# glmanhtu/vit-ed

Measured on AMD Instinct MI355X. Metric: patch-pairs/sec fwd+bwd, div2k_erosion7_4bin_patch8_64 ViT-ED, higher is better.
Workload: dtype bf16

## Files before the change

include/vited.h:

```cpp
#ifndef VITED_H
#define VITED_H

#include <stdint.h>

#ifdef __cplusplus
extern "C" {
#endif

#define VITED_ABI_VERSION 1

#define VITED_OK 0
#define VITED_ERR_BAD_ARG 1
#define VITED_ERR_UNSUPPORTED 2
#define VITED_ERR_LAUNCH 3
#define VITED_ERR_WORKSPACE 4

#define VITED_F32 0
#define VITED_BF16 1
#define VITED_F16 2
#define VITED_I32 3
#define VITED_I64 4

#define VITED_EPI_STORE 0
#define VITED_EPI_GELU 1
// ... 67 lines not shown
int64_t vited_layernorm_bwd_workspace_bytes(int64_t rows, int64_t dim);
int vited_layernorm_bwd(const void* dy, int dy_dtype, int64_t dy_ld, const float* x, int64_t x_ld,
                        const float* gamma, const float* mean, const float* rstd, const float* dx_in,
                        int64_t dx_in_ld, float* dx_out, int64_t dx_out_ld, void* dx_lp, int dx_lp_dtype,
                        int64_t dx_lp_ld, float* dgamma, float* dbeta, int accumulate, int64_t rows, int64_t dim,
                        float* workspace, int64_t workspace_bytes, void* stream);

int vited_layernorm_bwd_scaled(const void* dy, int dy_dtype, int64_t dy_ld, const float* x, int64_t x_ld,
                               const float* gamma, const float* mean, const float* rstd, const float* dx_in,
                               int64_t dx_in_ld, float* dx_out, int64_t dx_out_ld, void* dx_lp, int dx_lp_dtype,
                               int64_t dx_lp_ld, const float* lp_scale, float* dgamma, float* dbeta, int accumulate,
                               int64_t rows, int64_t dim, float* workspace, int64_t workspace_bytes, void* stream);

int vited_scale_rows_cast(const float* src, int64_t src_ld, const float* row_scale, void* dst, int dst_dtype, int64_t dst_ld,
                          int64_t rows, int64_t dim, void* stream);


int vited_gemm(const void* A, int64_t lda, const void* B, int64_t ldb, int b_layout, int dtype, int64_t M,
               int64_t N, int64_t K, int epilogue, const float* bias, const void* aux,
               const float* residual, void* out, void* out2, int64_t ldo, int64_t rows_per_batch,
               int64_t out_rows_per_batch, int64_t row_offset, int residual_bcast, void* stream);

int vited_gemm_scaled(const void* A, int64_t lda, const void* B, int64_t ldb, int b_layout, int dtype, int64_t M, int64_t N,
                      int64_t K, const float* bias, const float* residual, const float* row_scale, float* out, int64_t ldo,
                      void* stream);

int64_t vited_linear_bwd_weight_workspace_bytes(int64_t M, int64_t N, int64_t K);
int vited_linear_bwd_weight(const void* dY, int64_t lddy, const void* X, int64_t ldx, int dtype, int64_t M,
                            int64_t N, int64_t K, float* dW, float* dbias, int accumulate, float* workspace,
                            int64_t workspace_bytes, void* stream);

int vited_linear_bwd_weight_batched_supported(int count, const int64_t* M, const int64_t* N, const int64_t* K, int dtype);
int64_t vited_linear_bwd_weight_batched_workspace_bytes(int count, const int64_t* M, const int64_t* N, const int64_t* K);
int vited_linear_bwd_weight_batched(int count, const void* const* dY, const int64_t* lddy, const void* const* X,
                                    const int64_t* ldx, const int64_t* M, const int64_t* N, const int64_t* K, float* const* dW,
                                    float* const* dbias, int dtype, int accumulate, float* workspace, int64_t workspace_bytes,
                                    void* stream);

int vited_linear_layernorm_supported(int64_t M, int64_t N, int64_t K);

int vited_linear_residual_layernorm_fwd(const void* a, int64_t lda, const void* w, int64_t ldw, const float* bias,
                                        const float* residual, int64_t ldr, float* y, int64_t ldy, const float* gamma,
                                        const float* beta, float eps, void* h, int64_t ldh, float* mean, float* rstd,
                                        int64_t M, int64_t N, int64_t K, void* stream);

int vited_linear_residual_layernorm_fwd_scaled(const void* a, int64_t lda, const void* w, int64_t ldw, const float* bias,
                                               const float* residual, int64_t ldr, const float* row_scale, float* y, int64_t ldy,
                                               const float* gamma, const float* beta, float eps, void* h, int64_t ldh, float* mean,
                                               float* rstd, int64_t M, int64_t N, int64_t K, void* stream);

int vited_linear_layernorm_bwd_segmented(const void* dy, int64_t lddy, int64_t seg_k, int64_t seg_stride, int64_t segments,
                                         const void* wt, int64_t ldwt, const float* x, int64_t ldx, const float* gamma,
                                         const float* mean, const float* rstd, const float* dx_in, int64_t dx_in_ld,
                                         float* dx_out, int64_t dx_out_ld, void* dx_lp, int64_t dx_lp_ld, float* dgamma,
                                         float* dbeta, int accumulate, int64_t M, int64_t N, float* workspace,
                                         int64_t workspace_bytes, void* stream);
int64_t vited_linear_layernorm_bwd_partial_rows(int64_t M);
int vited_layernorm_bwd_finish_batched(int count, const float* const* partial, const int* nparts, float* const* dgamma,
                                       float* const* dbeta, const int* accumulate, int64_t dim, void* stream);
int64_t vited_linear_layernorm_bwd_workspace_bytes(int64_t M, int64_t N);
int vited_linear_layernorm_bwd(const void* dy, int64_t lddy, const void* wt, int64_t ldwt, const float* x, int64_t ldx,
                               const float* gamma, const float* mean, const float* rstd, const float* dx_in,
                               int64_t dx_in_ld, float* dx_out, int64_t dx_out_ld, void* dx_lp, int64_t dx_lp_ld,
                               float* dgamma, float* dbeta, int accumulate, int64_t M, int64_t N, int64_t K,
                               float* workspace, int64_t workspace_bytes, void* stream);

// ... 114 lines not shown
```

vit-ed_amd/csrc/gemm.hip:

```cpp
#include <stdlib.h>
#include <string.h>

#include "gemm_kernels.h"

static thread_local int g_last_gemm_path = 0;
extern "C" int vited_last_gemm_path(void) { return g_last_gemm_path; }

static int gemm_impl(const void* A, int64_t lda, const void* B, int64_t ldb, int b_layout, int dtype, int64_t M, int64_t N, int64_t K,
                     int epilogue, const float* bias, const void* aux, const float* residual, void* out, void* out2, int64_t ldo,
                     int64_t rows_per_batch, int64_t out_rows_per_batch, int64_t row_offset, int residual_bcast,
                     const float* row_scale, void* stream) {
    if (!A || !B || !out || M <= 0 || N <= 0 || K <= 0 || lda < K || ldo < N) return VITED_ERR_BAD_ARG;
    if (b_layout != VITED_B_NK && b_layout != VITED_B_KN) return VITED_ERR_BAD_ARG;
    if (ldb < (b_layout == VITED_B_NK ? K : N)) return VITED_ERR_BAD_ARG;
    if (epilogue < VITED_EPI_STORE || epilogue > VITED_EPI_GELU_GRAD) return VITED_ERR_BAD_ARG;
    if ((epilogue == VITED_EPI_GELU || epilogue == VITED_EPI_GELU_GRAD) && !out2) return VITED_ERR_BAD_ARG;
    if (epilogue == VITED_EPI_RESIDUAL && !residual) return VITED_ERR_BAD_ARG;
    if ((epilogue == VITED_EPI_MUL_GELU_GRAD || epilogue == VITED_EPI_MUL) && !aux) return VITED_ERR_BAD_ARG;
    if (rows_per_batch < 0 || (rows_per_batch > 0 && (out_rows_per_batch < rows_per_batch + row_offset || row_offset < 0)))
        return VITED_ERR_BAD_ARG;
    if (row_scale) {
        if (epilogue != VITED_EPI_RESIDUAL || rows_per_batch != 0) return VITED_ERR_BAD_ARG;
        epilogue = EPI_RESIDUAL_SCALED;
    }
// ... 75 lines not shown
        return rc;
    }
    g_last_gemm_path = 1;
    rc = gemm_tn_portable(dY, lddy, X, ldx, dtype, M, N, K, splits, slab, s);
    if (rc != VITED_OK) return rc;
    if (via_slabs) {
        rc = sum_rows_f32_single_pass(workspace, N * K, dW, splits, N * K, s, accumulate);
        if (rc != VITED_OK) return rc;
    }
    if (dbias) {
        float* ws2 = bias_tmp + N;
        const int64_t ws2_bytes = workspace_bytes - (splits * N * K + N) * (int64_t)sizeof(float);
        if (accumulate) {
            rc = vited_sum_rows(dY, dtype, lddy, bias_tmp, M, N, ws2, ws2_bytes, stream);
            if (rc == VITED_OK) rc = sum_rows_f32_single_pass(bias_tmp, N, dbias, 1, N, s, 1);
        } else {
            rc = vited_sum_rows(dY, dtype, lddy, dbias, M, N, ws2, ws2_bytes, stream);
        }
    }
    return rc;
}

extern "C" int vited_linear_bwd_weight_batched_supported(int count, const int64_t* M, const int64_t* N, const int64_t* K, int dtype) {
    return dtype == VITED_BF16 && gemm_tn_batch_supported(count, M, N, K) ? 1 : 0;
}

extern "C" int64_t vited_linear_bwd_weight_batched_workspace_bytes(int count, const int64_t* M, const int64_t* N, const int64_t* K) {
    if (!gemm_tn_batch_supported(count, M, N, K)) return 0;
    int64_t splits, ws, bs;
    gemm_tn_batch_layout(count, M, N, K, &splits, &ws, &bs);
    return splits * (ws + bs) * (int64_t)sizeof(float) + 256;
}

extern "C" int vited_linear_bwd_weight_batched(int count, const void* const* dY, const int64_t* lddy, const void* const* X,
                                               const int64_t* ldx, const int64_t* M, const int64_t* N, const int64_t* K,
                                               float* const* dW, float* const* dbias, int dtype, int accumulate, float* workspace,
                                               int64_t workspace_bytes, void* stream) {
    if (count < 1 || !dY || !lddy || !X || !ldx || !M || !N || !K || !dW || !dbias || !workspace) return VITED_ERR_BAD_ARG;
    if (dtype != VITED_BF16 || !gemm_tn_batch_supported(count, M, N, K)) return VITED_ERR_UNSUPPORTED;
    if (workspace_bytes < vited_linear_bwd_weight_batched_workspace_bytes(count, M, N, K)) return VITED_ERR_WORKSPACE;
    int64_t splits, ws, bs;
    gemm_tn_batch_layout(count, M, N, K, &splits, &ws, &bs);
    int has_bias[40];
    int64_t widths[40], nbias[40];
    for (int i = 0; i < count; ++i) {
        if (!dY[i] || !X[i] || !dW[i] || lddy[i] < N[i] || ldx[i] < K[i]) return VITED_ERR_BAD_ARG;
        has_bias[i] = dbias[i] != nullptr;
        widths[i] = N[i] * K[i];
        nbias[i] = N[i];
    }
    float* base = (float*)(((uintptr_t)workspace + 15) & ~(uintptr_t)15);
    float* slabs = base;
    float* bias_slabs = base + splits * ws;
    hipStream_t s = (hipStream_t)stream;
    g_last_gemm_path = 2;
    int rc = gemm_tn_batch(count, dY, lddy, X, ldx, M, N, K, has_bias, slabs, bias_slabs, s);
    if (rc != VITED_OK) return rc;
    return sum_slabs_batch(count, slabs, ws, bias_slabs, bs, splits, widths, dW, nbias, dbias, accumulate, s);
}
```

vit-ed_amd/csrc/gemm_kernels.h:

```cpp
#pragma once
#include "gemm_epilogue.h"

int gemm_portable(const void* A, int64_t lda, const void* B, int64_t ldb, int b_layout, int dtype, int64_t M, int64_t N,
                  int64_t K, int epilogue, const EpiParams& ep, hipStream_t s);
int gemm_tn_portable(const void* dY, int64_t lddy, const void* X, int64_t ldx, int dtype, int64_t M, int64_t N, int64_t K,
                     int64_t splits, float* out, hipStream_t s);

bool gemm_nt_mfma_supported(const void* A, int64_t lda, const void* B, int64_t ldb, int64_t M, int64_t N, int64_t K,
                            int epilogue, const EpiParams& ep);
int gemm_nt_mfma(const void* A, int64_t lda, const void* B, int64_t ldb, int64_t M, int64_t N, int64_t K, int epilogue,
                 const EpiParams& ep, hipStream_t s);
bool gemm_nt_areg_supported(int64_t ldw, int64_t M, int64_t N, int64_t K, int epilogue);
int gemm_nt_areg(const void* A, int64_t lda, const void* W, int64_t ldw, int64_t M, int64_t N, int epilogue, int waves,
                 const EpiParams& ep, hipStream_t s);
bool gemm_tn_mfma_supported(const void* dY, int64_t lddy, const void* X, int64_t ldx, int64_t M, int64_t N, int64_t K);
int64_t gemm_tn_mfma_splits(int64_t M, int64_t N, int64_t K);
int gemm_tn_mfma(const void* dY, int64_t lddy, const void* X, int64_t ldx, int64_t M, int64_t N, int64_t K, int64_t splits,
                 float* out, float* bias_out , hipStream_t s);

bool gemm_tn_batch_supported(int count, const int64_t* M, const int64_t* N, const int64_t* K);
void gemm_tn_batch_layout(int count, const int64_t* M, const int64_t* N, const int64_t* K, int64_t* splits, int64_t* slab_stride,
                          int64_t* bias_stride);
int gemm_tn_batch(int count, const void* const* dY, const int64_t* lddy, const void* const* X, const int64_t* ldx, const int64_t* M,
                  const int64_t* N, const int64_t* K, const int* has_bias, float* slabs, float* bias_slabs, hipStream_t s);
int sum_slabs_batch(int count, const float* slabs, int64_t slab_stride, const float* bias_slabs, int64_t bias_stride, int64_t splits,
                    const int64_t* widths, float* const* dW, const int64_t* nbias, float* const* dbias, int accumulate, hipStream_t s);

int sum_rows_f32_single_pass(const float* in, int64_t in_ld, float* out, int64_t batch, int64_t width, hipStream_t s,
                             int accumulate = 0);
int sum_slabs_pair(const float* in_a, int64_t ld_a, float* out_a, int64_t width_a, const float* in_b, int64_t ld_b, float* out_b,
                   int64_t width_b, int64_t batch, hipStream_t s, int accumulate);
```

vit-ed_amd/csrc/gemm_mfma.hip:

```cpp
#include <stdlib.h>

#include <mutex>

#include "gemm_kernels.h"
#include "gemm_nt_epilogue.h"
#include "gemm_lds.h"

template <int BKT, int WM, bool ASM_DMA = false>
__device__ __forceinline__ void nt_stage_load(const bf16* __restrict__ A, int64_t lda, const bf16* __restrict__ B,
                                              int64_t ldb, int64_t m0, int64_t n0, int64_t M, int64_t N, int64_t k0,
                                              char* stage, int wave, int lane) {
    using C = NtCfg<BKT, WM>;
    const int rsub = lane / C::CHUNKS, cp = lane % C::CHUNKS;
#ifndef NT_DBG_NO_A_DMA
#pragma unroll
    for (int i = 0; i < 32 / C::ROWS_PER_DMA; ++i) {
        const int r = wave * 32 + i * C::ROWS_PER_DMA + rsub;
        const int c = cp ^ C::swz(r);
        int64_t gm = m0 + r;
        gm = gm < M ? gm : M - 1;
        const bf16* asrc = A + gm * lda + k0 + c * 8;
        if constexpr (ASM_DMA) glds16_asm(asrc, stage + (wave * 32 + i * C::ROWS_PER_DMA) * C::ROW_BYTES);
        else glds16(asrc, stage + (wave * 32 + i * C::ROWS_PER_DMA) * C::ROW_BYTES);
    }
// ... 750 lines not shown
        status = hipFuncSetAttribute((const void*)gemm_tn_wide_kernel<true>, hipFuncAttributeMaxDynamicSharedMemorySize, LDS);
        if (status == hipSuccess)
            status = hipFuncSetAttribute((const void*)gemm_tn_wide_kernel<false>, hipFuncAttributeMaxDynamicSharedMemorySize, LDS);
    });
    if (status != hipSuccess) return VITED_ERR_LAUNCH;
    if (any_bias)
        hipLaunchKernelGGL((gemm_tn_wide_kernel<true>), dim3(b.total_tiles, (unsigned)splits), dim3(512), LDS, s, b, out, bias_out);
    else
        hipLaunchKernelGGL((gemm_tn_wide_kernel<false>), dim3(b.total_tiles, (unsigned)splits), dim3(512), LDS, s, b, out, bias_out);
    return VITED_OK;
}

static int launch_tn_wide(const void* dY, int64_t lddy, const void* X, int64_t ldx, int64_t M, int64_t N, int64_t K, int64_t splits,
                          float* out, float* bias_out, hipStream_t s) {
    TwBatch b = {};
    TwProblem& p = b.p[0];
    p.dY = (const bf16*)dY; p.X = (const bf16*)X; p.lddy = lddy; p.ldx = ldx; p.M = M;
    p.rows_per_split = ceil_div64(ceil_div64(M, splits), 32) * 32;
    p.N = (int)N; p.K = (int)K; p.tiles_k = (int)(K / 384); p.tile0 = 0; p.has_bias = bias_out != nullptr;
    b.count = 1;
    b.total_tiles = (int)ceil_div64(N, 128) * p.tiles_k;
    b.slab_stride = N * K;
    b.bias_stride = N;
    return launch_tn_wide_batch(b, splits, bias_out != nullptr, out, bias_out, s);
}

bool gemm_tn_batch_supported(int count, const int64_t* M, const int64_t* N, const int64_t* K) {
    if (count < 1 || count > TW_MAX_PROBLEMS) return false;
    for (int i = 0; i < count; ++i)
        if (!tn_use_wide(M[i], N[i], K[i]) || N[i] % 8 || N[i] > (1 << 20) || K[i] > (1 << 20)) return false;
    return true;
}

static inline int64_t tn_batch_splits(int count, const int64_t* M, const int64_t* N, const int64_t* K) {
    int64_t tiles = 0, mmin = M[0];
    for (int i = 0; i < count; ++i) {
        tiles += ceil_div64(N[i], 128) * (K[i] / 384);
        mmin = M[i] < mmin ? M[i] : mmin;
    }
    int64_t s = 256 / tiles;
    const int64_t max_s = ceil_div64(mmin, 256);
    if (s > max_s) s = max_s;
    return s < 1 ? 1 : s;
}

void gemm_tn_batch_layout(int count, const int64_t* M, const int64_t* N, const int64_t* K, int64_t* splits, int64_t* slab_stride,
                          int64_t* bias_stride) {
    *splits = tn_batch_splits(count, M, N, K);
    int64_t w = 0, b = 0;
    for (int i = 0; i < count; ++i) {
        w += N[i] * K[i];
        b += N[i];
    }
    *slab_stride = w;
    *bias_stride = b;
}

int gemm_tn_batch(int count, const void* const* dY, const int64_t* lddy, const void* const* X, const int64_t* ldx, const int64_t* M,
                  const int64_t* N, const int64_t* K, const int* has_bias, float* slabs, float* bias_slabs, hipStream_t s) {
    TwBatch b = {};
    int64_t splits;
    gemm_tn_batch_layout(count, M, N, K, &splits, &b.slab_stride, &b.bias_stride);
    int tile = 0;
    int64_t woff = 0, boff = 0;
    bool any_bias = false;
    for (int i = 0; i < count; ++i) {
        TwProblem& p = b.p[i];
        if (!gemm_tn_mfma_supported(dY[i], lddy[i], X[i], ldx[i], M[i], N[i], K[i])) return VITED_ERR_UNSUPPORTED;
        p.dY = (const bf16*)dY[i]; p.X = (const bf16*)X[i]; p.lddy = lddy[i]; p.ldx = ldx[i]; p.M = M[i];
        p.rows_per_split = ceil_div64(ceil_div64(M[i], splits), 32) * 32;
        p.N = (int)N[i]; p.K = (int)K[i]; p.tiles_k = (int)(K[i] / 384); p.tile0 = tile; p.has_bias = has_bias[i];
        p.slab_off = woff; p.bias_off = boff;
        tile += (int)ceil_div64(N[i], 128) * p.tiles_k;
        woff += N[i] * K[i];
        boff += N[i];
        any_bias = any_bias || has_bias[i];
    }
    b.count = count;
    b.total_tiles = tile;
    const int rc = launch_tn_wide_batch(b, splits, any_bias, slabs, bias_slabs, s);
    return rc != VITED_OK ? rc : vited_check_launch();
}

int gemm_tn_mfma(const void* dY, int64_t lddy, const void* X, int64_t ldx, int64_t M, int64_t N, int64_t K, int64_t splits,
                 float* out, float* bias_out, hipStream_t s) {
    int rc;
    if (tn_use_wide(M, N, K)) rc = launch_tn_wide(dY, lddy, X, ldx, M, N, K, splits, out, bias_out, s);
#if TN_FORCE_TM
    else rc = launch_tn<TN_FORCE_TM, TN_FORCE_STAGES>(dY, lddy, X, ldx, M, N, K, splits, out, bias_out, s);
#else
    else if (tn_use_ring(M, N, K)) rc = launch_tn<32, 3>(dY, lddy, X, ldx, M, N, K, splits, out, bias_out, s);
    else rc = launch_tn<64, 2>(dY, lddy, X, ldx, M, N, K, splits, out, bias_out, s);
#endif
    return rc != VITED_OK ? rc : vited_check_launch();
}
```

vit-ed_amd/functions.py:

```python
from __future__ import annotations

import contextlib
import os
from collections import namedtuple

import torch

from . import ops
from ._lib import (B_KN, B_NK, EPI_GELU_GRAD, EPI_MUL, EPI_RESIDUAL, EPI_STORE, EPI_STORE_F32)

LN_EPS = 1e-6


def _bundle(name, table):
    fields, keys = zip(*(pair.split('=') for pair in table.split()))
    return namedtuple(name, fields), keys


_ATTN = 'g1=norm1.weight b1=norm1.bias wqkv=attn.qkv.weight bqkv=attn.qkv.bias wproj=attn.proj.weight bproj=attn.proj.bias '
_CROSS = ('gc=norm_cross.weight bc=norm_cross.bias gx=norm_context.weight bx=norm_context.bias wq=cross_attn.q.weight '
          'bq=cross_attn.q.bias wkv=cross_attn.kv.weight bkv=cross_attn.kv.bias wcp=cross_attn.proj.weight bcp=cross_attn.proj.bias ')
_MLP = 'g2=norm2.weight b2=norm2.bias w1=mlp.fc1.weight bb1=mlp.fc1.bias w2=mlp.fc2.weight bb2=mlp.fc2.bias'
_PATCH = 'pw=patch_embed.proj.weight pb=patch_embed.proj.bias pos=pos_embed '
EncBlock, ENC_BLOCK_KEYS = _bundle('EncBlock', _ATTN + _MLP)
DecBlock, DEC_BLOCK_KEYS = _bundle('DecBlock', _ATTN + _CROSS + _MLP)
EncShared, ENC_SHARED_KEYS = _bundle('EncShared', _PATCH)
DecShared, DEC_SHARED_KEYS = _bundle('DecShared', _PATCH + 'cls=cls_token gN=norm.weight bN=norm.bias wh=head.weight bh=head.bias')


def split_params(params, shared_type, block_type):
    ns, nb = len(shared_type._fields), len(block_type._fields)
    if len(params) < ns or (len(params) - ns) % nb:
        raise ValueError(f'{len(params)} parameters are not {ns} shared + a whole number of {nb}-parameter blocks')
    return shared_type._make(params[:ns]), [block_type._make(params[i: i + nb]) for i in range(ns, len(params), nb)]


def flatten_params(shared, blocks):
# ... 150 lines not shown
        return tuple(self.get(i, j) for j in range(self.per_sample.shape[1]))


def _take_drop_rows(rt, which, nblk, nbr, batch, n, device, cls_block=None):
    dp = rt.drop_path
    if dp is None or dp[which] is None:
        return None
    scales, live = dp[which], dp[2][which]
    if not any(any(row) for row in live):
        return None
    if tuple(scales.shape) != (nblk, nbr, batch) or scales.dtype != torch.float32 or scales.device != device:
        raise ValueError(f'drop-path scales: expected fp32 {(nblk, nbr, batch)} on {device}, got {scales.dtype} {tuple(scales.shape)} on '
                         f'{scales.device}')
    return _DropRows(scales.contiguous(), live, n, cls_block)


def _gtarget(rt, p):
    if p is None or not rt.direct_grads:
        return None
    g = p.grad
    if g is None or g.dtype != torch.float32 or not g.is_contiguous() or g.shape != p.shape or g.device != p.device:
        return None
    return g


def _ln_bwd(rt, dy, x, gamma, beta, mean, rstd, **kw):
    gg, gb = _gtarget(rt, gamma), _gtarget(rt, beta)
    if gg is not None and gb is not None:
        dx, dx_lp, _, _ = ops.layernorm_bwd(dy, x, gamma, mean, rstd, dgamma=gg, dbeta=gb, **kw)
        return dx, dx_lp, None, None
    return ops.layernorm_bwd(dy, x, gamma, mean, rstd, **kw)


def _weight_grads(rt, dy, x_saved, w, b):
    if rt.keep_cam:
        return None, None
    gw = _gtarget(rt, w)
    gb = _gtarget(rt, b) if b is not None else None
    direct = gw is not None and (b is None or gb is not None)
    q = rt.dw_queue
    if q is not None and dy.dtype == torch.bfloat16 and dy.shape[0] >= 4096 and x_saved.shape[1] % 384 == 0:
        if direct:
            q.append((dy, x_saved, gw.view(gw.shape[0], -1), gb, True))
            return None, None
        dw = torch.empty((dy.shape[1], x_saved.shape[1]), dtype=torch.float32, device=dy.device)
        db = torch.empty(dy.shape[1], dtype=torch.float32, device=dy.device) if b is not None else None
        q.append((dy, x_saved, dw, db, False))
        return dw.view_as(w), db
    if direct:
        ops.linear_bwd_weight(dy, x_saved, want_bias=b is not None, dw_out=gw.view(gw.shape[0], -1), db_out=gb)
        return None, None
    dw, db = ops.linear_bwd_weight(dy, x_saved)
    return dw.view_as(w), (db if b is not None else None)


class _DwBatch:

    ROUND = 256

    def __init__(self, rt, kind=None):
        self.rt, self.blocks, self.kind = rt, rt.group_dw, kind

    def __enter__(self):
        self.outer = self.rt.dw_queue
        self.rt.dw_queue = [] if (self.rt.batch_dw and not self.rt.exact) else None
        self.mark = 0
        return self

    @contextlib.contextmanager
    def block(self):
        yield
        self._end_of_block()

    @staticmethod
    def _tiles(items):
        return sum(-(-dy.shape[1] // 128) * (x.shape[1] // 384) for dy, x, _dw, _db, _a in items)

    def _end_of_block(self):
        q = self.rt.dw_queue
        if q is None:
            return
        if not self.blocks:
            self.flush()
            return
        this, count = self._tiles(q[self.mark:]), len(q) - self.mark
        self.mark = len(q)
        if self._tiles(q) + this > self.ROUND or len(q) + count > ops.MAX_BATCHED_WEIGHT_GRADS:
            self.flush()

    def flush(self):
        q = self.rt.dw_queue
        if not q:
            return
        self.rt.dw_queue, self.mark = [], 0
        with _BlockSpan(self.rt, self.kind, len(q), 'dw'):
            for acc in (True, False):
                _launch_weight_grads([(dy, x, dw, db) for dy, x, dw, db, a in q if a == acc], acc)

    def __exit__(self, exc_type, *exc):
        if exc_type is None:
            self.flush()
        self.rt.dw_queue = self.outer
        return False


def _launch_weight_grads(items, accumulate):
    for i in range(0, len(items), ops.MAX_BATCHED_WEIGHT_GRADS):
        part = items[i: i + ops.MAX_BATCHED_WEIGHT_GRADS]
        if len(part) > 1 and ops.linear_bwd_weight_batched(part, accumulate):
            continue
        for dy, x, dw, db in part:
            if accumulate:
                ops.linear_bwd_weight(dy, x, want_bias=db is not None, dw_out=dw, db_out=db)
                continue
            got_w, got_b = ops.linear_bwd_weight(dy, x, want_bias=db is not None)
            dw.copy_(got_w)
            if db is not None:
                db.copy_(got_b)


def _linear_bwd(rt, dy, x_saved, w, b=None, aux=None):
    wt, layout = rt.weight_t(w)
    if aux is not None:
        dx = ops.gemm(dy, wt, b_layout=layout, epilogue=EPI_MUL, aux=aux)
    else:
        dx = ops.gemm(dy, wt, b_layout=layout)
    dw, db = _weight_grads(rt, dy, x_saved, w, b)
    return dx, dw, db


def _row_kernel_ok(rt, m, n, k, dtype, *rowwise):
    return (rt.fused_ln and not rt.exact and ops.linear_layernorm_supported(m, n, k, dtype)
            and all(t is None or (t.dim() == 2 and t.stride(1) == 1 and t.stride(0) % 4 == 0) for t in rowwise))


def _res_linear(rt, a, w, bias, residual, ln=None, scale=None):
# ... 183 lines not shown
    def forward(ctx, rt: Runtime, img, *params):
        shared, blocks = split_params(params, EncShared, EncBlock)
        grad = any(ctx.needs_input_grad)
        x, patches, batch, n = _patch_tokens_fwd(rt, img, shared, with_cls=False)
        drop = _take_drop_rows(rt, 0, len(blocks), 2, batch, n, x.device)
        tape = []
        ln1 = None
        for i, P in enumerate(blocks):
            s_attn, s_mlp = drop.block(i) if drop is not None else (None, None)
            chain = _hand_over_ln(rt, x, P, grad or s_mlp is not None)
            with _BlockSpan(rt, 'enc', i, 'fwd'):
                xa, sa, ln2 = _attn_branch_fwd(rt, x, P, batch, n, key=('blocks', i, 'attn'), ln=ln1, next_ln=(P.g2, P.b2) if chain else None,
                                               scale=s_attn)
                xb, sm, ln1 = _mlp_fwd(rt, xa, P, grad, ln=ln2, next_ln=_norm1_of(blocks, i + 1) if chain else None, scale=s_mlp)
            if grad:
                tape.append((x, sa, xa, sm))
            x = xb
            if rt.tap is not None:
                rt.tap[f'enc.x.{len(tape) - 1 if grad else 0}'] = x.clone()
        if grad:
            ctx.rt, ctx.tape, ctx.patches, ctx.batch, ctx.params = rt, tape, patches, batch, (shared, blocks)
            ctx.drop = drop
        return x.view(batch, n, rt.dim)

    @staticmethod
    def backward(ctx, dout):
        rt, batch, n = ctx.rt, ctx.batch, ctx.rt.n1
        shared, blocks = ctx.params
        dx = dout.contiguous().view(batch * n, rt.dim).float()
        drop = ctx.drop
        scale_of = (lambda i, j: drop.get(i, j)) if drop is not None else (lambda i, j: None)
        dx_lp = _lp_scaled(rt, dx, scale_of(len(blocks) - 1, 1))
        gblocks = [None] * len(blocks)
        with _ln_sums(rt), _DwBatch(rt, kind='enc') as dwg:
            for i in reversed(range(len(blocks))):
                x, sa, xa, sm = ctx.tape[i]
                ctx.tape[i] = None
                with _BlockSpan(rt, 'enc', i, 'bwd'), dwg.block():
                    dx, dx_lp, gm = _mlp_bwd(rt, dx, dx_lp, xa, blocks[i], sm, lp_scale=scale_of(i, 0))
                    dx, dx_lp, ga = _attn_branch_bwd(rt, dx, dx_lp, x, blocks[i], sa, batch, n, key=('blocks', i, 'attn'),
                                                     lp_scale=scale_of(i - 1, 1))
                if rt.tap is not None:
                    rt.tap[f'enc.dx.{i}'] = dx.clone()
                gblocks[i] = EncBlock(**ga, **gm)
        gshared = EncShared(**_patch_tokens_bwd(rt, dx, ctx.patches, shared, with_cls=False, batch=batch))
        ctx.tape = ctx.patches = ctx.drop = None
        return (None, None, *_cam_only(rt, flatten_params(gshared, gblocks)))


def _dense_rows(t):
    out = torch.empty(t.shape, dtype=t.dtype, device=t.device)
    out.copy_(t)
    return out


def _dec_self_fwd(rt, x, P, batch, n, cls_only, key=None, ln1=None, fuse_ln=True, scale=None):
    next_ln = (P.gc, P.bc) if fuse_ln else None
    if not cls_only:
        return _attn_branch_fwd(rt, x, P, batch, n, key=key, ln=ln1, next_ln=next_ln, scale=scale)
    d = rt.dim
    h1, m1, r1 = ln1 if ln1 is not None else ops.layernorm_fwd(x, P.g1, P.b1, LN_EPS, rt.act_dtype)
    qkv = ops.gemm(h1, rt.weight(P.wqkv), bias=P.bqkv)
    qkv3 = qkv.view(batch, n, 3 * d)
    o0, lse0 = ops.attention_fwd(qkv3[:, 0:1, 0:d], qkv3[:, :, d:2 * d], qkv3[:, :, 2 * d:3 * d], rt.heads, rt.scale)
    o0 = o0.view(batch, d)
    x0 = _dense_rows(x.view(batch, n, d)[:, 0, :])
    xa, lnq = _res_linear(rt, o0, P.wproj, P.bproj, x0, next_ln, scale)
# ... 150 lines not shown
                                                    [g.detach() for g in gs], [b.detach() for b in bes], out=bufs)
    xhat, mean, rstd = ops.layernorm_fwd(ctxf, rt._unit_ln[0], rt._unit_ln[1], LN_EPS, rt.act_dtype)
    n2 = 2 * rt.dim
    kv_all = torch.empty((len(blocks), ctxf.shape[0], n2), dtype=rt.act_dtype, device=dev)
    for l in range(len(blocks)):
        ops.gemm(xhat, bufs[0][l * n2:(l + 1) * n2], bias=bufs[2][l * n2:(l + 1) * n2], out=kv_all[l])
    return kv_all, (xhat, mean, rstd), bufs


def _context_kv_folded_bwd(rt, dkv_all, ctxf, saved, bufs, blocks):
    xhat, mean, rstd = saved
    ones = rt._unit_ln[0]
    nblk, mc, n2 = dkv_all.shape
    if _row_kernel_ok(rt, mc, bufs[1].shape[0], nblk * n2, dkv_all.dtype, ctxf):
        dctx, _, _, _ = ops.linear_layernorm_bwd(dkv_all, bufs[1], ctxf, ones, mean, rstd)
    else:
        dh = torch.zeros((mc, rt.dim), dtype=torch.float32, device=ctxf.device)
        for l in range(nblk):
            dh = ops.gemm(dkv_all[l], bufs[1][:, l * n2:(l + 1) * n2], epilogue=EPI_RESIDUAL, residual=dh)
        dctx, _, _, _ = ops.layernorm_bwd(dh, ctxf, ones, mean, rstd)
    dwf = torch.empty((nblk * n2, rt.dim), dtype=torch.float32, device=ctxf.device)
    dbf = torch.empty(nblk * n2, dtype=torch.float32, device=ctxf.device)
    _launch_weight_grads([(dkv_all[l], xhat, dwf[l * n2:(l + 1) * n2], dbf[l * n2:(l + 1) * n2]) for l in range(nblk)], False)
    ws, bs, gs, bes = _kv_params(blocks)
    targets = [(_gtarget(rt, w), _gtarget(rt, b) if b is not None else None, _gtarget(rt, g), _gtarget(rt, be)) for w, b, g, be in zip(ws, bs, gs, bes)]
    direct = all(tw is not None and tg is not None and tbe is not None and (b is None or tb is not None) for (tw, tb, tg, tbe), b in zip(targets, bs))
    if not direct:
        targets = [(torch.empty_like(w), torch.empty_like(b) if b is not None else None, torch.empty_like(g), torch.empty_like(be))
                   for w, b, g, be in zip(ws, bs, gs, bes)]
    ops.unfold_context_grads(dwf, dbf, [w.detach() for w in ws], [g.detach() for g in gs], [b.detach() for b in bes],
                             [tw for tw, _, _, _ in targets], [tb for _, tb, _, _ in targets], [tg for _, _, tg, _ in targets],
                             [tbe for _, _, _, tbe in targets], accumulate=direct)
    return dctx, [dict.fromkeys(('gx', 'bx', 'wkv', 'bkv')) if direct else dict(gx=tg, bx=tbe, wkv=tw, bkv=tb) for tw, tb, tg, tbe in targets]


class DecoderFn(torch.autograd.Function):
    @staticmethod
    def forward(ctx, rt: Runtime, feats, img2, img2_index, img1_index, *params):
        shared, blocks = split_params(params, DecShared, DecBlock)
        grad = any(ctx.needs_input_grad)
        x, patches, batch, n = _patch_tokens_fwd(rt, img2, shared, with_cls=True, batch_index=img2_index)
        seg = img1_index
        b1 = batch if seg is None else seg.items
        if seg is not None:
            if rt.keep_attn or rt.keep_cam:
                raise NotImplementedError('the attention-map paths (keep_attn / keep_cam) take gathered features, not an image-1 index')
            assert seg.index.numel() == batch, f'{seg.index.numel()} image-1 indices for {batch} image-2 samples'
        assert feats.shape == (b1, rt.n1, rt.dim), f'features {tuple(feats.shape)} do not match {b1} context items'
        ctxf = feats.detach().contiguous().float().view(b1 * rt.n1, rt.dim)
        tape = []
        d = rt.dim
        cls_tail = rt.cls_tail and rt.c_depth > 0 and not (rt.keep_attn or rt.keep_cam)
        drop = _take_drop_rows(rt, 1, len(blocks), 3, batch, n, x.device, cls_block=rt.c_depth - 1 if cls_tail else None)
        ln1 = None
        fold = rt.fold_context and not rt.exact and rt.c_depth > 1 and rt.c_depth <= ops.MAX_FOLDED_BLOCKS and rt.dim % 32 == 0
        kv_all = kv_saved = fold_bufs = None
        if fold:
            kv_all, kv_saved, fold_bufs = _context_kv_folded(rt, ctxf, blocks)
        for i, P in enumerate(blocks):
            x, entry, ln1 = _dec_block_fwd(rt, x, ctxf, P, batch, n, grad, cls_tail and i == rt.c_depth - 1, index=i, ln1=ln1,
                                           next_ln=_norm1_of(blocks, i + 1), kv3=kv_all[i].view(b1, rt.n1, 2 * d) if fold else None,
                                           scales=drop.block(i) if drop is not None else (None, None, None), seg=seg)
            if grad:
                tape.append(entry)
            if rt.tap is not None:
                rt.tap[f'dec.x.{i}'] = x.clone()
# ... 17 lines not shown
        dl = _lp(rt, dlogits.contiguous().float())
        wh_act = rt.weight(shared.wh)
        dy = ops.gemm(dl, wh_act, b_layout=B_KN)
        dwh, dbh = _weight_grads(rt, dl, y, shared.wh, shared.bh)
        drop, last = ctx.drop, len(blocks) - 1
        seg = ctx.seg
        b1 = batch if seg is None else seg.items
        scale_of = (lambda i, j: drop.get(i, j)) if drop is not None else (lambda i, j: None)
        s_head = drop.per_sample[last, 2] if drop is not None and drop.live[last][2] else None
        if s_head is not None:
            lp_dtype = rt.act_dtype
            if ctx.cls_tail:
                dx, dx_lp, dgN, dbN = _ln_bwd(rt, dy, xcls, shared.gN, shared.bN, mN, rN, lp_scale=s_head, lp_dtype=lp_dtype)
            else:
                dx = torch.zeros((batch * n, d), dtype=torch.float32, device=dy.device)
                dx_lp = torch.zeros((batch * n, d), dtype=lp_dtype, device=dy.device)
                _, _, dgN, dbN = _ln_bwd(rt, dy, xcls, shared.gN, shared.bN, mN, rN, dx_out=dx.view(batch, n, d)[:, 0, :],
                                         dx_lp=dx_lp.view(batch, n, d)[:, 0, :], lp_scale=s_head, lp_dtype=lp_dtype)
        elif ctx.cls_tail:
            dx, dx_lp, dgN, dbN = _ln_bwd(rt, dy, xcls, shared.gN, shared.bN, mN, rN, want_lp=not rt.exact)
        else:
            dx = torch.zeros((batch * n, d), dtype=torch.float32, device=dy.device)
            dx_lp = dx_lp3 = None
            if not rt.exact:
                dx_lp = torch.zeros((batch * n, d), dtype=rt.act_dtype, device=dy.device)
                dx_lp3 = dx_lp.view(batch, n, d)[:, 0, :]
            _, _, dgN, dbN = _ln_bwd(rt, dy, xcls, shared.gN, shared.bN, mN, rN, dx_out=dx.view(batch, n, d)[:, 0, :], dx_lp=dx_lp3)
        if rt.exact and s_head is None:
            dx_lp = dx
        dctx = None
        gblocks = [None] * len(blocks)
        dkv_all = torch.empty_like(ctx.fold[0]) if ctx.fold is not None else None
        with _ln_sums(rt):
            with _DwBatch(rt, kind='dec') as dwg:
                for i in reversed(range(len(blocks))):
                    entry = ctx.tape[i]
                    ctx.tape[i] = None
                    with dwg.block():
                        dx, dx_lp, dctx, gblocks[i] = _dec_block_bwd(rt, dx, dx_lp, ctx.ctxf, dctx, blocks[i], entry, batch, n,
                                                                     ctx.cls_tail and i == rt.c_depth - 1, i,
                                                                     dkv3=dkv_all[i].view(b1, rt.n1, 2 * d) if dkv_all is not None else None,
                                                                     lp_scales=(scale_of(i, 1), scale_of(i, 0), scale_of(i - 1, 2)), seg=seg)
                    if rt.tap is not None:
                        rt.tap[f'dec.dx.{i}'] = dx.clone()
                        if dctx is not None:
                            rt.tap[f'dec.dctx.{i}'] = dctx.clone()
            if dkv_all is not None:
                dctx, kv_grads = _context_kv_folded_bwd(rt, dkv_all, ctx.ctxf, ctx.fold[1], ctx.fold[2], blocks)
                gblocks = [g._replace(**kv) for g, kv in zip(gblocks, kv_grads)]
                ctx.fold = None
        gshared = DecShared(**_patch_tokens_bwd(rt, dx, ctx.patches, shared, with_cls=True, batch=batch), gN=dgN, bN=dbN, wh=dwh, bh=dbh)
        dfeats = dctx.view(b1, rt.n1, d) if ctx.feats_needs_grad and dctx is not None else None
        ctx.tape = ctx.patches = ctx.ctxf = ctx.final = ctx.drop = ctx.seg = None
        return (None, dfeats, None, None, None, *_cam_only(rt, flatten_params(gshared, gblocks)))
```

vit-ed_amd/ops.py:

```python
from __future__ import annotations

import ctypes as C
from typing import NamedTuple

import torch

from . import _lib
from ._lib import (B_KN, B_NK, BF16, EPI_GELU, EPI_GELU_GRAD, EPI_MUL, EPI_MUL_GELU_GRAD, EPI_RESIDUAL, EPI_STORE, EPI_STORE_F32, F16,
                   F32, I32, I64)

_DTYPE = {torch.float32: F32, torch.bfloat16: BF16, torch.float16: F16, torch.int32: I32, torch.int64: I64}
_FLOATS = (torch.float32, torch.bfloat16, torch.float16)


def _code(dtype: torch.dtype) -> int:
    if dtype not in (torch.float32, torch.bfloat16):
        raise TypeError(f'vited ops support float32 and bfloat16 activations, got {dtype}')
    return _DTYPE[dtype]


def _need_gpu(*tensors):
    for t in tensors:
        if t is not None and not t.is_cuda:
            raise RuntimeError('vited ops run on the MI355X HIP kernels only: got a CPU tensor '
                               '(there is no CPU fallback; the fp32 CPU oracle lives in oracle/ for tests)')


def _ptr(t):
    return 0 if t is None else t.data_ptr()


def _stream():
    return torch.cuda.current_stream().cuda_stream


# ... 379 lines not shown
    ws = _scratch(_lib.load().vited_linear_bwd_weight_workspace_bytes(m, n, k), x.device)
    _lib.call('vited_linear_bwd_weight', _ptr(dy), lddy, _ptr(x), ldx, _code(x.dtype), m, n, k, _ptr(dw), _ptr(db), int(accumulate), *ws,
              _stream())
    return dw, db


MAX_BATCHED_WEIGHT_GRADS = 40


def linear_bwd_weight_batched(items, accumulate: bool) -> bool:
    n = len(items)
    if n < 1 or n > MAX_BATCHED_WEIGHT_GRADS:
        return False
    for dy, x, dw, db in items:
        _need_gpu(dy, x, dw, db)
        if dy.dtype != torch.bfloat16 or x.dtype != torch.bfloat16 or dy.shape[0] != x.shape[0]:
            return False
        assert dw.dtype == torch.float32 and dw.is_contiguous() and dw.numel() == dy.shape[1] * x.shape[1]
        assert db is None or (db.dtype == torch.float32 and db.is_contiguous() and db.numel() == dy.shape[1])
        if dw.data_ptr() % 16 or (db is not None and db.data_ptr() % 16) or dy.data_ptr() % 16 or x.data_ptr() % 16:
            return False
    dys, xs, dws, dbs = zip(*items)
    M = _host_array(C.c_int64, [dy.shape[0] for dy in dys])
    N = _host_array(C.c_int64, [dy.shape[1] for dy in dys])
    K = _host_array(C.c_int64, [x.shape[1] for x in xs])
    lib = _lib.load()
    if not lib.vited_linear_bwd_weight_batched_supported(n, M, N, K, BF16):
        return False
    lddy, ldx = _host_array(C.c_int64, map(_rows2d, dys)), _host_array(C.c_int64, map(_rows2d, xs))
    ws = _scratch(lib.vited_linear_bwd_weight_batched_workspace_bytes(n, M, N, K), dys[0].device)
    _lib.call('vited_linear_bwd_weight_batched', n, _host_array(C.c_void_p, dys), lddy, _host_array(C.c_void_p, xs), ldx, M, N, K,
              _host_array(C.c_void_p, dws), _host_array(C.c_void_p, dbs), BF16, int(bool(accumulate)), *ws, _stream())
    return True


def linear_layernorm_supported(m: int, n: int, k: int, dtype: torch.dtype) -> bool:
    return dtype == torch.bfloat16 and bool(_lib.load().vited_linear_layernorm_supported(int(m), int(n), int(k)))


def linear_residual_layernorm_fwd(a, w, bias, residual, gamma=None, beta=None, eps: float = 1e-6, out=None, row_scale=None):
    _need_gpu(a, w, bias, residual, gamma, beta, out, row_scale)
    assert a.dtype == w.dtype == torch.bfloat16 and residual.dtype == torch.float32
    lda, ldw, ldr = _rows2d(a), _rows2d(w), _rows2d(residual)
    m, k = a.shape
    n = w.shape[0]
    assert w.shape[1] == k and residual.shape == (m, n)
    y = out if out is not None else torch.empty((m, n), dtype=torch.float32, device=a.device)
    assert y.dtype == torch.float32 and y.shape == (m, n)
    h = mean = rstd = None
    if gamma is not None:
        h = torch.empty((m, n), dtype=torch.bfloat16, device=a.device)
        mean = torch.empty(m, dtype=torch.float32, device=a.device)
        rstd = torch.empty(m, dtype=torch.float32, device=a.device)
    tail = (_ptr(y), _rows2d(y), _ptr(gamma), _ptr(beta), float(eps), _ptr(h), n, _ptr(mean), _ptr(rstd), m, n, k, _stream())
    if row_scale is not None:
        _check_row_scale(row_scale, m)
        _lib.call('vited_linear_residual_layernorm_fwd_scaled', _ptr(a), lda, _ptr(w), ldw, _ptr(bias), _ptr(residual), ldr, _ptr(row_scale),
                  *tail)
    else:
        _lib.call('vited_linear_residual_layernorm_fwd', _ptr(a), lda, _ptr(w), ldw, _ptr(bias), _ptr(residual), ldr, *tail)
    return y, h, mean, rstd


def linear_layernorm_bwd(dy, wt, x, gamma, mean, rstd, dx_in=None, dx_out=None, want_lp: bool = False, dgamma=None, dbeta=None,
                         defer=None, lp_scale=None):
    _need_gpu(dy, wt, x, gamma, mean, rstd, dx_in, dx_out, lp_scale)
# ... 558 lines not shown
```

Before: 43670.

## Plan batched weight-grad flush groups with DP over announced per-block shapes

Adds a C entry point that reports the batched weight-gradient tile geometry. On the Python side, the encoder and decoder backward passes announce each block's weight-grad shapes up front. A dynamic program then picks where to flush the queued dW GEMMs, balancing wave occupancy (split-K count per 256-slot round) against the cost of slab reduction, in place of the previous greedy tile-count threshold. If the observed shapes diverge from the announcement, it falls back to the greedy rule. Risks are extra host-side planning overhead and mismatches between announced and actual shapes.

```diff
diff --git a/include/vited.h b/include/vited.h
--- a/include/vited.h
+++ b/include/vited.h
@@ -123,6 +123,8 @@
 
 int vited_linear_bwd_weight_batched_supported(int count, const int64_t* M, const int64_t* N, const int64_t* K, int dtype);
 int64_t vited_linear_bwd_weight_batched_workspace_bytes(int count, const int64_t* M, const int64_t* N, const int64_t* K);
+int vited_linear_bwd_weight_batched_layout(int count, const int64_t* M, const int64_t* N, const int64_t* K, int64_t* tiles,
+                                           int64_t* splits, int64_t* round, int64_t* min_split_rows);
 int vited_linear_bwd_weight_batched(int count, const void* const* dY, const int64_t* lddy, const void* const* X,
                                     const int64_t* ldx, const int64_t* M, const int64_t* N, const int64_t* K, float* const* dW,
                                     float* const* dbias, int dtype, int accumulate, float* workspace, int64_t workspace_bytes,
diff --git a/vit-ed_amd/csrc/gemm.hip b/vit-ed_amd/csrc/gemm.hip
--- a/vit-ed_amd/csrc/gemm.hip
+++ b/vit-ed_amd/csrc/gemm.hip
@@ -131,6 +131,19 @@
     return splits * (ws + bs) * (int64_t)sizeof(float) + 256;
 }
 
+extern "C" int vited_linear_bwd_weight_batched_layout(int count, const int64_t* M, const int64_t* N, const int64_t* K, int64_t* tiles,
+                                                      int64_t* splits, int64_t* round, int64_t* min_split_rows) {
+    if (!M || !N || !K || !tiles || !splits || !round || !min_split_rows) return VITED_ERR_BAD_ARG;
+    if (!gemm_tn_batch_supported(count, M, N, K)) return VITED_ERR_UNSUPPORTED;
+    int64_t ws, bs;
+    TnBatchGeometry g;
+    gemm_tn_batch_layout(count, M, N, K, splits, &ws, &bs, &g);
+    *tiles = g.tiles;
+    *round = g.round;
+    *min_split_rows = g.min_split_rows;
+    return VITED_OK;
+}
+
 extern "C" int vited_linear_bwd_weight_batched(int count, const void* const* dY, const int64_t* lddy, const void* const* X,
                                                const int64_t* ldx, const int64_t* M, const int64_t* N, const int64_t* K,
                                                float* const* dW, float* const* dbias, int dtype, int accumulate, float* workspace,
diff --git a/vit-ed_amd/csrc/gemm_kernels.h b/vit-ed_amd/csrc/gemm_kernels.h
--- a/vit-ed_amd/csrc/gemm_kernels.h
+++ b/vit-ed_amd/csrc/gemm_kernels.h
@@ -19,8 +19,13 @@
                  float* out, float* bias_out , hipStream_t s);
 
 bool gemm_tn_batch_supported(int count, const int64_t* M, const int64_t* N, const int64_t* K);
+struct TnBatchGeometry {
+    int64_t tiles;
+    int64_t round;
+    int64_t min_split_rows;
+};
 void gemm_tn_batch_layout(int count, const int64_t* M, const int64_t* N, const int64_t* K, int64_t* splits, int64_t* slab_stride,
-                          int64_t* bias_stride);
+                          int64_t* bias_stride, TnBatchGeometry* geometry = nullptr);
 int gemm_tn_batch(int count, const void* const* dY, const int64_t* lddy, const void* const* X, const int64_t* ldx, const int64_t* M,
                   const int64_t* N, const int64_t* K, const int* has_bias, float* slabs, float* bias_slabs, hipStream_t s);
 int sum_slabs_batch(int count, const float* slabs, int64_t slab_stride, const float* bias_slabs, int64_t bias_stride, int64_t splits,
diff --git a/vit-ed_amd/csrc/gemm_mfma.hip b/vit-ed_amd/csrc/gemm_mfma.hip
--- a/vit-ed_amd/csrc/gemm_mfma.hip
+++ b/vit-ed_amd/csrc/gemm_mfma.hip
@@ -806,20 +806,28 @@
     return true;
 }
 
+#define TW_TILE_N 128
+#define TW_TILE_K 384
+#define TW_ROUND 256
+#define TW_MIN_SPLIT_ROWS 256
+
+static inline int64_t tn_batch_tiles(int count, const int64_t* N, const int64_t* K) {
+    int64_t tiles = 0;
+    for (int i = 0; i < count; ++i) tiles += ceil_div64(N[i], TW_TILE_N) * (K[i] / TW_TILE_K);
+    return tiles;
+}
+
 static inline int64_t tn_batch_splits(int count, const int64_t* M, const int64_t* N, const int64_t* K) {
-    int64_t tiles = 0, mmin = M[0];
-    for (int i = 0; i < count; ++i) {
-        tiles += ceil_div64(N[i], 128) * (K[i] / 384);
-        mmin = M[i] < mmin ? M[i] : mmin;
-    }
-    int64_t s = 256 / tiles;
-    const int64_t max_s = ceil_div64(mmin, 256);
+    int64_t mmin = M[0];
+    for (int i = 0; i < count; ++i) mmin = M[i] < mmin ? M[i] : mmin;
+    int64_t s = TW_ROUND / tn_batch_tiles(count, N, K);
+    const int64_t max_s = ceil_div64(mmin, TW_MIN_SPLIT_ROWS);
     if (s > max_s) s = max_s;
     return s < 1 ? 1 : s;
 }
 
 void gemm_tn_batch_layout(int count, const int64_t* M, const int64_t* N, const int64_t* K, int64_t* splits, int64_t* slab_stride,
-                          int64_t* bias_stride) {
+                          int64_t* bias_stride, TnBatchGeometry* geometry) {
     *splits = tn_batch_splits(count, M, N, K);
     int64_t w = 0, b = 0;
     for (int i = 0; i < count; ++i) {
@@ -828,6 +836,7 @@
     }
     *slab_stride = w;
     *bias_stride = b;
+    if (geometry) *geometry = {tn_batch_tiles(count, N, K), TW_ROUND, TW_MIN_SPLIT_ROWS};
 }
 
 int gemm_tn_batch(int count, const void* const* dY, const int64_t* lddy, const void* const* X, const int64_t* ldx, const int64_t* M,
@@ -845,7 +854,7 @@
         p.rows_per_split = ceil_div64(ceil_div64(M[i], splits), 32) * 32;
         p.N = (int)N[i]; p.K = (int)K[i]; p.tiles_k = (int)(K[i] / 384); p.tile0 = tile; p.has_bias = has_bias[i];
         p.slab_off = woff; p.bias_off = boff;
-        tile += (int)ceil_div64(N[i], 128) * p.tiles_k;
+        tile += (int)ceil_div64(N[i], TW_TILE_N) * p.tiles_k;
         woff += N[i] * K[i];
         boff += N[i];
         any_bias = any_bias || has_bias[i];
diff --git a/vit-ed_amd/functions.py b/vit-ed_amd/functions.py
--- a/vit-ed_amd/functions.py
+++ b/vit-ed_amd/functions.py
@@ -1,8 +1,10 @@
 from __future__ import annotations
 
 import contextlib
+import functools
 import os
 from collections import namedtuple
+from fractions import Fraction
 
 import torch
 
@@ -219,6 +221,40 @@
     return ops.layernorm_bwd(dy, x, gamma, mean, rstd, **kw)
 
 
+def _dw_queued(rt, dy, x):
+    return rt.dw_queue is not None and dy.dtype == torch.bfloat16 and dy.shape[0] >= 4096 and x.shape[1] % 384 == 0
+
+
+def _dw_shapes(rt, linears):
+    return tuple((m, w.shape[0], w[0].numel()) for m, w in linears if m >= 4096 and w[0].numel() % 384 == 0)
+
+
+def plan_dw_groups(tiles, products, max_splits, round_slots=256, max_products=40, slab_cost=0):
+    n = len(tiles)
+
+    def group(lo, hi):
+        t = sum(tiles[lo:hi])
+        if hi - lo > 1 and sum(products[lo:hi]) > max_products:
+            return None
+        if t == 0:
+            return Fraction(0), 0, 1
+        if t > round_slots:
+            return Fraction(-(-t // round_slots)), t, 1
+        s = max(1, min(round_slots // t, min(m for m, ti in zip(max_splits[lo:hi], tiles[lo:hi]) if ti)))
+        return Fraction(1, s) + (slab_cost * Fraction(s * t, round_slots) if s > 1 else 0), t, s
+
+    best = [(Fraction(0), 0, [])] + [None] * n
+    for j in range(1, n + 1):
+        for i in range(j):
+            g = group(i, j)
+            if g is None:
+                continue
+            cand = (best[i][0] + g[0], best[i][1] + (g[1] > 0))
+            if best[j] is None or cand <= best[j][:2]:
+                best[j] = cand + (best[i][2] + [(j - i, g[1], g[2])],)
+    return best[n][2]
+
+
 def _weight_grads(rt, dy, x_saved, w, b):
     if rt.keep_cam:
         return None, None
@@ -226,7 +262,7 @@
     gb = _gtarget(rt, b) if b is not None else None
     direct = gw is not None and (b is None or gb is not None)
     q = rt.dw_queue
-    if q is not None and dy.dtype == torch.bfloat16 and dy.shape[0] >= 4096 and x_saved.shape[1] % 384 == 0:
+    if _dw_queued(rt, dy, x_saved):
         if direct:
             q.append((dy, x_saved, gw.view(gw.shape[0], -1), gb, True))
             return None, None
@@ -243,15 +279,15 @@
 
 class _DwBatch:
 
-    ROUND = 256
-
-    def __init__(self, rt, kind=None):
-        self.rt, self.blocks, self.kind = rt, rt.group_dw, kind
+    def __init__(self, rt, kind=None, announced=None):
+        self.rt, self.blocks, self.kind, self.announced = rt, rt.group_dw, kind, announced
 
     def __enter__(self):
         self.outer = self.rt.dw_queue
         self.rt.dw_queue = [] if (self.rt.batch_dw and not self.rt.exact) else None
-        self.mark = 0
+        self.mark, self.done, self.ends = 0, 0, None
+        if self.rt.dw_queue is not None and self.blocks and self.announced is not None:
+            self.ends = _dw_group_ends(tuple(tuple(sorted(b)) for b in self.announced))
         return self
 
     @contextlib.contextmanager
@@ -260,8 +296,8 @@
         self._end_of_block()
 
     @staticmethod
-    def _tiles(items):
-        return sum(-(-dy.shape[1] // 128) * (x.shape[1] // 384) for dy, x, _dw, _db, _a in items)
+    def _shapes(items):
+        return tuple(sorted((dy.shape[0], dy.shape[1], x.shape[1]) for dy, x, _dw, _db, _a in items))
 
     def _end_of_block(self):
         q = self.rt.dw_queue
@@ -270,9 +306,19 @@
         if not self.blocks:
             self.flush()
             return
-        this, count = self._tiles(q[self.mark:]), len(q) - self.mark
+        this = q[self.mark:]
         self.mark = len(q)
-        if self._tiles(q) + this > self.ROUND or len(q) + count > ops.MAX_BATCHED_WEIGHT_GRADS:
+        if not this and self.ends is None:
+            return
+        if self.ends is not None:
+            if self.done < len(self.announced) and self._shapes(this) == tuple(sorted(self.announced[self.done])):
+                self.done += 1
+                if self.done in self.ends:
+                    self.flush()
+                return
+            self.ends = None
+        lay, nxt = ops.linear_bwd_weight_batched_layout(self._shapes(q)), ops.linear_bwd_weight_batched_layout(self._shapes(this))
+        if lay is None or nxt is None or lay.tiles + nxt.tiles > lay.round or len(q) + len(this) > ops.MAX_BATCHED_WEIGHT_GRADS:
             self.flush()
 
     def flush(self):
@@ -289,6 +335,23 @@
             self.flush()
         self.rt.dw_queue = self.outer
         return False
+
+
+@functools.lru_cache(maxsize=64)
+def _dw_group_ends(announced):
+    lays = [ops.linear_bwd_weight_batched_layout(b) if b else ops.WeightGradLayout(0, 1, 0, 1) for b in announced]
+    live = [l for l in lays if l is not None and l.tiles]
+    if any(l is None for l in lays) or not live:
+        return None
+    rows = min(m for b in announced for m, _n, _k in b)
+    groups = plan_dw_groups([l.tiles for l in lays], [len(b) for b in announced],
+                            [-(-min(m for m, _n, _k in b) // l.min_split_rows) if b else 1 for b, l in zip(announced, lays)],
+                            round_slots=live[0].round, max_products=ops.MAX_BATCHED_WEIGHT_GRADS, slab_cost=Fraction(1024, rows))
+    ends, at = set(), 0
+    for blocks, _tiles, _splits in groups:
+        at += blocks
+        ends.add(at)
+    return frozenset(ends)
 
 
 def _launch_weight_grads(items, accumulate):
@@ -538,7 +601,9 @@
         scale_of = (lambda i, j: drop.get(i, j)) if drop is not None else (lambda i, j: None)
         dx_lp = _lp_scaled(rt, dx, scale_of(len(blocks) - 1, 1))
         gblocks = [None] * len(blocks)
-        with _ln_sums(rt), _DwBatch(rt, kind='enc') as dwg:
+        rows = batch * n
+        announced = [_dw_shapes(rt, [(rows, P.w2), (rows, P.w1), (rows, P.wproj), (rows, P.wqkv)]) for P in reversed(blocks)]
+        with _ln_sums(rt), _DwBatch(rt, kind='enc', announced=announced) as dwg:
             for i in reversed(range(len(blocks))):
                 x, sa, xa, sm = ctx.tape[i]
                 ctx.tape[i] = None
@@ -755,6 +820,16 @@
                              [tw for tw, _, _, _ in targets], [tb for _, tb, _, _ in targets], [tg for _, _, tg, _ in targets],
                              [tbe for _, _, _, tbe in targets], accumulate=direct)
     return dctx, [dict.fromkeys(('gx', 'bx', 'wkv', 'bkv')) if direct else dict(gx=tg, bx=tbe, wkv=tw, bkv=tb) for tw, tb, tg, tbe in targets]
+
+
+def _dec_dw_announced(rt, blocks, batch, n, items, cls_tail, folded):
+    out = []
+    for i in reversed(range(len(blocks))):
+        P, rows = blocks[i], batch * n
+        r = batch if cls_tail and i == rt.c_depth - 1 else rows
+        kv = [] if folded else [(items * rt.n1, P.wkv)]
+        out.append(_dw_shapes(rt, [(r, P.w2), (r, P.w1), (r, P.wcp), (r, P.wq), *kv, (r, P.wproj), (rows, P.wqkv)]))
+    return out
 
 
 class DecoderFn(torch.autograd.Function):
@@ -838,7 +913,7 @@
         gblocks = [None] * len(blocks)
         dkv_all = torch.empty_like(ctx.fold[0]) if ctx.fold is not None else None
         with _ln_sums(rt):
-            with _DwBatch(rt, kind='dec') as dwg:
+            with _DwBatch(rt, kind='dec', announced=_dec_dw_announced(rt, blocks, batch, n, b1, ctx.cls_tail, dkv_all is not None)) as dwg:
                 for i in reversed(range(len(blocks))):
                     entry = ctx.tape[i]
                     ctx.tape[i] = None
diff --git a/vit-ed_amd/ops.py b/vit-ed_amd/ops.py
--- a/vit-ed_amd/ops.py
+++ b/vit-ed_amd/ops.py
@@ -1,6 +1,7 @@
 from __future__ import annotations
 
 import ctypes as C
+import functools
 from typing import NamedTuple
 
 import torch
@@ -446,6 +447,24 @@
     _lib.call('vited_linear_bwd_weight_batched', n, _host_array(C.c_void_p, dys), lddy, _host_array(C.c_void_p, xs), ldx, M, N, K,
               _host_array(C.c_void_p, dws), _host_array(C.c_void_p, dbs), BF16, int(bool(accumulate)), *ws, _stream())
     return True
+
+
+class WeightGradLayout(NamedTuple):
+    tiles: int
+    splits: int
+    round: int
+    min_split_rows: int
+
+
+@functools.lru_cache(maxsize=None)
+def linear_bwd_weight_batched_layout(shapes) -> WeightGradLayout | None:
+    if not 1 <= len(shapes) <= MAX_BATCHED_WEIGHT_GRADS:
+        return None
+    M, N, K = (_host_array(C.c_int64, [int(s[i]) for s in shapes]) for i in range(3))
+    out = [C.c_int64() for _ in range(4)]
+    if _lib.load().vited_linear_bwd_weight_batched_layout(len(shapes), M, N, K, *map(C.byref, out)) != 0:
+        return None
+    return WeightGradLayout(*(int(v.value) for v in out))
 
 
 def linear_layernorm_supported(m: int, n: int, k: int, dtype: torch.dtype) -> bool:
```

Result: no change. 43890 (median of 6 runs) (+0.5%).
